# Enigmatisms/AdaPT

Hardware: AMD Instinct MI355X
Metric: Msamples/s (W*H*spp/s), unidirectional MIS path tracing (higher is better)
Workload: dtype f32

## Files before the change

adapt_amd/_lib.py:

```python
from __future__ import annotations

import ctypes as C
import os

_HERE = os.path.dirname(os.path.abspath(__file__))
LIB_PATHS = {"fast": os.environ.get("ADAPT_MI_LIB") or os.path.join(_HERE, "libadapt_mi.so"),
             "exact": os.environ.get("ADAPT_MI_LIB_EXACT") or os.path.join(_HERE, "libadapt_mi_exact.so")}
_variant = "exact" if os.environ.get("APT_EXACT", "0") not in ("", "0") else "fast"
LIB_PATH = LIB_PATHS[_variant]

f32p = C.POINTER(C.c_float)
i32p = C.POINTER(C.c_int32)
u32p = C.POINTER(C.c_uint32)
u8p = C.POINTER(C.c_uint8)
f64p = C.POINTER(C.c_double)
APT_N_KERNELS = 5
KERNEL_NAMES = ("generate", "extend", "shade", "shadow", "finalize")


class AptError(RuntimeError):
    pass


class SceneDesc(C.Structure):
# ... 85 lines not shown
    "apt_stream": (C.c_int, [C.c_void_p, C.POINTER(C.c_void_p)]),
    "apt_intersect": (C.c_int, [C.c_void_p, C.c_int32, f32p, f32p, i32p, f32p, f32p]),
    "apt_occluded": (C.c_int, [C.c_void_p, C.c_int32, f32p, f32p, f32p, i32p]),
    "apt_rng_stream": (C.c_int, [C.c_int32, C.c_uint32, C.c_uint32, C.c_uint32, C.c_int32, u32p]),
    "apt_bxdf_probe": (C.c_int, [C.c_int32, C.c_int32, i32p, f32p, f32p, C.c_float, C.c_int32, C.c_uint32, f32p]),
    "apt_medium_probe": (C.c_int, [C.c_int32, C.c_int32, i32p, f32p, C.c_int32, f32p, C.c_uint32, f32p]),
    "apt_volume_probe": (C.c_int, [C.c_int32, C.c_int32, i32p, f32p, f32p, C.c_int32, f32p, C.c_uint32, f32p]),
    "apt_emitter_probe": (C.c_int, [C.c_void_p, C.c_int32, f32p, C.c_uint32, f32p]),
    "apt_texture_probe": (C.c_int, [C.c_void_p, C.c_int32, i32p, f32p, f32p]),
    "apt_surface_maps_probe": (C.c_int, [C.c_void_p, C.c_int32, i32p, f32p, f32p]),
    "apt_transient_bin_probe": (C.c_int, [C.c_int32, C.c_int32, f32p, C.c_float, C.c_float, C.c_int32, i32p]),
    "apt_renderer_info": (C.c_int, [C.c_void_p, i32p, i32p, C.POINTER(C.c_int64), i32p, C.POINTER(C.c_char_p), i32p]),
    "apt_renderer_camera_fused": (C.c_int, [C.c_void_p, i32p]),
    "apt_renderer_light_strips": (C.c_int, [C.c_void_p, i32p]),
    "apt_renderer_record_staged": (C.c_int, [C.c_void_p, i32p]),
    "apt_measure_sclk_mhz": (C.c_int, [C.c_int32, f32p]),
    "apt_last_error": (C.c_char_p, []),
    "apt_version": (C.c_char_p, []),
}

_libs = {}


def use(variant: str) -> str:
    global _variant, LIB_PATH
    if variant not in LIB_PATHS:
        raise ValueError(f"unknown build variant {variant!r}")
    prev, _variant = _variant, variant
    LIB_PATH = LIB_PATHS[variant]
    return prev
# ... 36 lines not shown
```

adapt_amd/csrc/api.hip:

```cpp
#include <hip/hip_runtime.h>
#include <chrono>

#include <algorithm>
#include <cmath>
#include <cstdio>
#include <cstdlib>
#include <cstring>
#include <limits>
#include <memory>
#include <string>
#include <vector>

#include "../../include/adapt_mi.h"
#include "bvh_build.hpp"
#include "shade_stage.hpp"
#include "unit_kernels.hpp"
#include "aov.hpp"
#include "volumetric.hpp"

#define APT_EXPORT extern "C" __attribute__((visibility("default")))

static thread_local std::string g_err;
static int fail(int code, const std::string& msg) { g_err = msg; return code; }
#define HIP_TRY(expr)                                                                              \
    do {                                                                                           \
        hipError_t e_ = (expr);                                                                    \
        if (e_ != hipSuccess)                                                                      \
            return fail(APT_E_HIP, std::string(#expr) + ": " + hipGetErrorString(e_));             \
    } while (0)

typedef void (*shade_fn)(DevScene, Params, Queues, Counters*, ShadeIn, int, int);
typedef void (*shade_traced_fn)(DevScene, Params, Queues, Counters*, int, int);
typedef void (*shade_cam_fn)(DevScene, Params, Queues, Counters*, const unsigned long long*);
typedef void (*shade_tr_fn)(DevScene, Params, Queues, Counters*, ShadeIn, int, int, TransQ);
struct ShadeVariant { int bm, sm; const char* name; shade_fn fn; shade_tr_fn transient; shade_traced_fn traced; shade_cam_fn traced_cam; shade_traced_fn traced_staged; };
#if APT_FAST
#define APT_FLAT_FN(...) __VA_ARGS__
#else
#define APT_FLAT_FN(...) nullptr
#endif
#define APT_TRACED_PAIR(STEM, ...) APT_FLAT_FN(STEM<__VA_ARGS__>), APT_FLAT_FN(STEM##_cam<__VA_ARGS__>)
#define APT_TRACED_PLAIN(BM, SM, TEX) APT_TRACED_PAIR(k_shade_traced, BM, SM, TEX), nullptr
#define APT_TRACED_LEAN(BM, SM, TEX) APT_TRACED_PAIR(k_shade_traced_lean, BM, SM), APT_FLAT_FN(k_shade_traced_lean_staged<BM, SM>)
#define APT_SHADE_VARIANT(BM, SM, TEX, NAME, TRACED) {BM, SM, NAME, k_shade<BM, SM, TEX>, k_shade_tr<BM, SM, TEX>, APT_TRACED_##TRACED(BM, SM, TEX)}
static const ShadeVariant kShadeVariants[] = {
    APT_SHADE_VARIANT(APT_BX_LAMBERTIAN, APT_SRC_POINT, 0, "lambertian/point", LEAN),
    APT_SHADE_VARIANT(APT_BX_BLINN_PHONG | APT_BX_LAMBERTIAN, APT_SRC_POINT_AREA, 0, "phong+lambertian/point+area", PLAIN),
    APT_SHADE_VARIANT(APT_BX_BLINN_PHONG | APT_BX_LAMBERTIAN | APT_BX_MIRROR | APT_BX_GLASS, APT_SRC_POINT_AREA, 0, "phong+lambertian+mirror+glass/point+area", PLAIN),
    APT_SHADE_VARIANT(APT_BX_ALL, APT_SRC_ALL, 0, "all models", PLAIN),
};
static const ShadeVariant kTexturedShade = APT_SHADE_VARIANT(APT_BX_ALL, APT_SRC_ALL, 1, "all models + image textures", PLAIN);
struct ClassDef { int mask; const char* name; int group, slot, vgroup, vslot; };
constexpr int APT_N_GROUPS = 2, APT_N_VGROUPS = 3, APT_VGROUP_SLOTS = 4;
static constexpr ClassDef kClass[] = {
    {APT_BX_LAMBERTIAN, "lambertian", 0, 0, 0, 0},
    {APT_BX_BLINN_PHONG, "blinn-phong", 1, 0, 2, 0},
    {APT_BX_OREN_NAYAR, "oren-nayar", 1, 1, 0, 1},
    {APT_BX_MIRROR | APT_BX_GLASS | APT_BX_NULL, "delta", 0, 1, 0, 2},
// ... 134 lines not shown
enum Pipeline { PIPE_STAGED, PIPE_SORTED, PIPE_TRACED, PIPE_VOLUMETRIC };

struct apt_renderer {
    const apt_scene* scene = nullptr;
    apt_render_cfg cfg{};
    Params par{};
    int n_cols = 0, npix = 0, spp_batch = 1;
    int cnt = 0;
    std::vector<Lane> lanes;
    int n_lanes = 1;
    hipStream_t stream() const { return lanes[0].stream; }
    DevBuf accum, scratch, pix_key;
    DevBuf cam_strips;
    int record_stage = 0;
    shade_traced_fn traced_fn = nullptr;
    int camera_fuse = 0;
    int light_strips = 0;
    Counters host_counters{};
    int grid_small = 0, grid_trace = 0, nq = APT_MAX_NQ;
    const ShadeVariant* shade = nullptr;
    int trace_mode = TRACE_BVH;
    int trace_nt = BLOCK;
    int trace_items = BLOCK;
    Pipeline pipeline = PIPE_STAGED;
    int dyn_fetch = 0;
    bool tile_ok = false;
    extend_fn extend = nullptr, fix = nullptr;
    int ovf_levels = 0;
    int n_cq = 0;
    int vev_single = 0;
// ... 526 lines not shown
    if (textured) r->shade = &kTexturedShade;
    const char* env_sorted = getenv("APT_SORTED");
    const bool fits = sc->n_classes <= APT_MAX_CLASSES;
    const bool sorted = !textured && fits && (env_sorted ? (atoi(env_sorted) != 0 && sc->n_classes >= 1) : sc->n_classes >= 2);
    bool want_traced = true;
    if (const char* f = getenv("APT_FUSED")) {
        const int want = atoi(f);
        if (want == 1) fprintf(stderr, "adapt_mi: APT_FUSED=1 (light samples only traced in place) was retired in round 5; running the staged pipeline (APT_FUSED=0). Use 2 for rays traced in place.\n");
        want_traced = want >= 2;
    }
    const bool can_trace = r->trace_mode == TRACE_FLAT && S == 1 && !r->split() && r->shade->traced != nullptr;
    r->pipeline = c.volumetric ? PIPE_VOLUMETRIC : (sorted ? PIPE_SORTED : ((can_trace && want_traced) ? PIPE_TRACED : PIPE_STAGED));
    p.traced = (r->pipeline == PIPE_TRACED) ? 1 : 0;
    const bool want_stage = !(getenv("APT_RECORD_STAGE") && atoi(getenv("APT_RECORD_STAGE")) == 0);
    r->record_stage = (p.traced && want_stage && r->shade->traced_staged != nullptr) ? 1 : 0;
    r->traced_fn = r->record_stage ? r->shade->traced_staged : r->shade->traced;
    p.nee_vm = (!c.volumetric && !r->split() && r->trace_mode == TRACE_FLAT && S > 1) ? 1 : 0;
    p.l_planes = (!p.nee_vm && S >= 2 && S <= 4) ? S : 1;
    if (r->pipeline == PIPE_VOLUMETRIC) {
        if (c.max_bounce > 255) { return fail(APT_E_INVALID, "apt_renderer_create: the volumetric tracer keeps the bounce count in 8 bits (max_bounce <= 255)"); }
        if (!sc->has_aabb) { return fail(APT_E_INVALID, "apt_renderer_create: the volumetric tracer needs the object boxes (world bound)"); }
        r->vev_single = (textured || sc->n_classes + 1 > APT_MAX_CLASSES) ? 1 : 0;
        const int n_surf = r->vev_single ? 1 : sc->n_classes;
        r->n_cq = n_surf + 1;
        const int smi = vgroup_emitter_set(sc->src_mask), vi = sc->has_volume ? 1 : 0;
        r->vev_all = kVEventAll[smi][vi];
        for (size_t o = 0; o < sc->obj_class.size(); o++)
            if (!sc->obj_null[o]) r->vev_live[r->vev_single ? 0 : sc->obj_class[o]] = true;
        r->vev_live[n_surf] = true;
        for (int g = 0; g < APT_N_VGROUPS; g++) { r->vgroup_fn[g] = kVGroup[smi][vi][g]; for (int k = 0; k < APT_VGROUP_SLOTS; k++) r->vgroup_cls[g][k] = -1; }
        if (!r->vev_single) for (int c = 0; c < n_surf; c++) if (r->vev_live[c]) r->vgroup_cls[kClass[sc->class_def[c]].vgroup][kClass[sc->class_def[c]].vslot] = c;
// ... 524 lines not shown
    const int batch_cap = lane_batch(r, n_spp);
    while (done < n_spp) {
        const int B = (n_spp - done < batch_cap) ? (n_spp - done) : batch_cap;
        Lane& ln = r->lanes[(size_t)(batch % r->n_lanes)];
        hipStream_t st = ln.stream;
        const Queues& q = ln.q;
        Counters* cnt = ln.cnt();
        Params p = r->par; p.cnt_base = r->cnt; p.spp_batch = B;
        const size_t total = (size_t)r->npix * (size_t)B;
        if (int rc = begin_batch(r, ln)) return rc;
#if APT_FAST
        if (r->pipeline == PIPE_TRACED) {
            const unsigned long long* strips = r->cam_strips.as<unsigned long long>();
            int cur = 0, b0 = 0;
            if (r->camera_fuse) {
                { LaunchTimer t(r, APT_K_SHADE, st); hipLaunchKernelGGL(r->shade->traced_cam, dim3(grid_for(total, r->grid_small, nq)), dim3(BLOCK), 0, st, sc, p, q, cnt, strips); }
                { LaunchTimer t(r, APT_K_SHADE, st); hipLaunchKernelGGL(r->traced_fn, dim3(r->grid_fix), dim3(BLOCK), 0, st, sc, p, q, cnt, 0, 0); }
                cur = 1; b0 = 1;
            } else {
                LaunchTimer t(r, APT_K_GENERATE, st);
                if (r->adaptive) hipLaunchKernelGGL(k_generate_trace_ad, dim3(grid_for(total, r->grid_small, 1)), dim3(BLOCK), 0, st, sc, p, q, cnt, (const uint8_t*)r->aq.active, strips);
                else hipLaunchKernelGGL(k_generate_trace, dim3(grid_for(total, r->grid_small, 1)), dim3(BLOCK), 0, st, sc, p, q, cnt, strips);
            }
            for (int b = b0; b < p.max_bounce; b++) {
                { LaunchTimer t(r, APT_K_SHADE, st); hipLaunchKernelGGL(r->traced_fn, dim3(grid_for(total, r->grid_small, nq)), dim3(BLOCK), 0, st, sc, p, q, cnt, cur, b); }
                cur ^= 1;
            }
            if (p.max_bounce > 0) { LaunchTimer t(r, APT_K_SHADOW, st, false); hipLaunchKernelGGL(r->fix, dim3(r->grid_fix), dim3(BLOCK), 0, st, sc, p, q, cnt, cur, (const uint32_t*)cnt->n_active[cur], ln.plan); }
        } else
#endif
        {
// ... 593 lines not shown
APT_EXPORT int apt_renderer_camera_fused(const apt_renderer* r, int32_t* out) {
    if (!r || !out) return fail(APT_E_INVALID, "apt_renderer_camera_fused: null argument");
    *out = r->camera_fuse;
    return APT_OK;
}
APT_EXPORT int apt_renderer_light_strips(const apt_renderer* r, int32_t* out) {
    if (!r || !out) return fail(APT_E_INVALID, "apt_renderer_light_strips: null argument");
    *out = r->light_strips;
    return APT_OK;
}
APT_EXPORT int apt_renderer_record_staged(const apt_renderer* r, int32_t* out) {
    if (!r || !out) return fail(APT_E_INVALID, "apt_renderer_record_staged: null argument");
    *out = r->record_stage;
    return APT_OK;
}
APT_EXPORT int apt_renderer_info(const apt_renderer* r, int32_t* spp_batch, int32_t* n_subqueues, int64_t* queue_bytes, int32_t* lds_bytes, const char** shade_variant, int32_t* trace_mode) {
    if (!r) return fail(APT_E_INVALID, "apt_renderer_info: null handle");
    if (spp_batch) *spp_batch = r->spp_batch;
    if (n_subqueues) *n_subqueues = r->nq;
    if (queue_bytes) *queue_bytes = (int64_t)r->lanes[0].pool.bytes * (int64_t)r->lanes.size();
    if (lds_bytes) *lds_bytes = (int32_t)r->lds_bytes;
    if (shade_variant) *shade_variant = r->shade_name.c_str();
    if (trace_mode) *trace_mode = r->trace_mode;
    return APT_OK;
}
```

adapt_amd/csrc/shade_stage.hpp:

```cpp
#pragma once
#include "stages.hpp"

APT_D float ti_fmod(float a, float b) { float q = floorf(a / b); return a - b * q; }
APT_D f3 mix3(f3 a, f3 b, float t) { return a * (1.0f - t) + b * t; }
APT_D f3 texture_query(const DevScene& sc, int map, int obj, float u, float v) {
    const int* ti_ = sc.tex_i + 15 * obj + 5 * map; const float* tf = sc.tex_f + 6 * obj + 2 * map;
    const float w = (float)ti_[3], h = (float)ti_[4];
    const float scaled_u = ti_fmod((u * tf[0]) * w, w - 1.f), scaled_v = ti_fmod((v * tf[1]) * h, h - 1.f);
    float floor_u = floorf(scaled_u), floor_v = floorf(scaled_v);
    const float ratio_u = fmaxf(scaled_u - floor_u, 0.f), ratio_v = fmaxf(scaled_v - floor_v, 0.f);
    floor_u = fminf(fmaxf(floor_u, 0.f), w - 1.f); floor_v = fminf(fmaxf(floor_v, 0.f), h - 1.f);
    const float ceil_u = fminf(floor_u + 1.f, w - 1.f), ceil_v = fminf(floor_v + 1.f, h - 1.f);
    const int fu = (int)(floor_u + (float)ti_[1]), fv = (int)(floor_v + (float)ti_[2]), cu = (int)(ceil_u + (float)ti_[1]), cv = (int)(ceil_v + (float)ti_[2]);
    const float* img = sc.atlas[map]; const int W = sc.atlas_w[map];
    const float* r0 = img + (size_t)fv * W * 3; const float* r1 = img + (size_t)cv * W * 3;
    const f3 q_ff = ld3(r0 + 3 * fu), q_cf = ld3(r0 + 3 * cu), q_fc = ld3(r1 + 3 * fu), q_cc = ld3(r1 + 3 * cu);
    return mix3(mix3(q_ff, q_cf, ratio_u), mix3(q_fc, q_cc, ratio_u), ratio_v);
}
APT_D bool get_uv_item(const DevScene& sc, int map, int obj, int prim, float bu, float bv, f3& out) {
    if (sc.atlas[map] == nullptr || !(sc.tex_i[15 * obj + 5 * map] > -255)) return false;
    const float* uv = sc.uvs + 6 * prim;
    const float w0 = 1.f - bu - bv;
    const float gu = (uv[2] * bu + uv[4] * bv) + uv[0] * w0, gv = (uv[3] * bu + uv[5] * bv) + uv[1] * w0;
    out = texture_query(sc, map, obj, gu, gv);
// ... 185 lines not shown
    ls.contrib = (c * (A_->p).inv_S) * vx.thr;
    ls.want = !(ls.contrib.x == 0.f && ls.contrib.y == 0.f && ls.contrib.z == 0.f);
    return ls;
}
template <int BM, int SM, typename R, typename Gather>
APT_D f3 emit_and_scatter(const ShadeArgs3* A_, Vertex& vx, R& rng, float& new_pdf, bool& is_spec, Gather&& gather) {
    if ((SM & APT_SRC_AREA) && vx.hit_light >= 0) {
        const f3 emit_int = emitter_eval_le((A_->sc).src[vx.hit_light], vx.hit_point - vx.o, vx.it.n_s);
        if (!(emit_int.x == 0.f && emit_int.y == 0.f && emit_int.z == 0.f)) gather((emit_int * vx.emission_weight) * vx.thr);
    }
    f3 spec;
    const f3 new_d = surface_sample<BM>(vx.bx, vx.it, vx.d, (A_->sc).world_ior, (A_->p).two_sides, rng, spec, new_pdf, is_spec);
    vx.thr = vx.thr * fdiv3(spec, new_pdf);
    return new_d;
}
APT_D void shadow_store(const Queues& q, uint32_t so, f3 o, f3 dir, float dist, f3 contrib) {
    st3q(q.sh_o, q.sh_cap, so, o); st3q(q.sh_d, q.sh_cap, so, dir); stq(q.sh_tmax, so, dist); st3q(q.sh_c, q.sh_cap, so, contrib);
}
struct ShadeTally { uint32_t shade, shadow, poison; };
APT_D void tally_flush(const ShadeTally& t, const uint32_t* s_draws, Counters* cnt, int sq) {
    flush_uniform(t.shade, &cnt->stats[sq][ST_SHADE]);
    flush_uniform(t.shadow, &cnt->stats[sq][ST_SHADOW]);
    if (lane_id() == 0 && s_draws[threadIdx.x >> 6]) atomicAdd(&cnt->stats[sq][ST_DRAWS], (unsigned long long)s_draws[threadIdx.x >> 6]);
    flush_uniform(t.poison, &cnt->stats[sq][ST_POISON]);
}
#if APT_FAST
template <int BM, int SM, int TEX, bool CAM = false, bool STAGE = false>
APT_D void shade_traced(args3_ptr A0, Counters* cnt, int cur_, int bounce_, const unsigned long long* strips = nullptr) {
    static_assert(!(CAM && STAGE), "a camera-fed row loads no record");
    const ShadeArgs3* A_ = args_fresh(A0);
    const int cur = CAM ? 0 : cur_, bounce = CAM ? 0 : bounce_;
    const int nxt = cur ^ 1;
    const SubLoop sl = sub_loop((A_->p).nq);
    const uint32_t qbase = (uint32_t)sl.q * (A_->p).subcap, sh_qbase = (uint32_t)sl.q * (A_->q).sh_subcap;
    uint32_t* next_counter = &cnt->n_tr[(bounce + 1) % 3][0][sl.q * CNT_PAD];
    if (sl.first == 0 && threadIdx.x == 0) {
        cnt->n_tr[(bounce + 2) % 3][0][sl.q * CNT_PAD] = 0;
        cnt->n_tr[(bounce + 2) % 3][(A_->q).tr_ncls][sl.q * CNT_PAD] = 0;
    }
    const EmitterGeom geom = {(A_->sc).precom, (A_->sc).normals, (A_->sc).obj_info};
    __shared__ uint32_t s_draws[BLOCK / 64];
    if (lane_id() == 0) s_draws[threadIdx.x >> 6] = 0;
    ShadeTally tl = {0u, 0u, 0u};
    uint32_t t_traced = 0, t_lit = 0, t_extend = 0, t_samples = 0;
// ... 48 lines not shown
#ifdef APT_ROWTOP_STATS
    t_loop0 = __builtin_amdgcn_s_memtime();
#endif
    for (uint32_t base = sl.first; base < n; base += sl.stride) {
        APT_ARGS_PHASE();
        const uint32_t pos = base + threadIdx.x, idx = qbase + pos;
        bool alive = pos < n;
        const uint32_t cu_pm = pf_pm;
        float4 cu_ra = make_float4(0.f, 0.f, 0.f, 0.f), cu_rb = cu_ra;
        if (PFP) { const int rp = max(tr_prim(cu_pm), 0); cu_ra = (A_->sc).prim_shade[2 * rp]; cu_rb = (A_->sc).prim_shade[2 * rp + 1]; prefetch_prim(base + sl.stride); }
        Vertex vx; vertex_reset(vx);
        Rng rng; rng_init(rng, 0u, 0u, 0u, 0u);
        f3 Lc = splat3(0.f);
        bool entry = alive;
        float ray_pdf = 1.f;
        if constexpr (CAM) {
            const uint32_t w = (uint32_t)__builtin_amdgcn_readfirstlane((int)(pos >> 6)) * (uint32_t)(A_->p).nq + (uint32_t)sl.q;
            const uint32_t id_ = w * 64u + lane_id();
            const bool valid = alive && id_ < cam_total;
            f3 dir = mk3(0.f, 0.f, 1.f);
            uint32_t draws = 0;
            uint32_t jitter_tail[2] = {0u, 0u};
            if (valid) {
                const uint32_t lp = id_ % (uint32_t)(A_->p).npix, s = id_ / (uint32_t)(A_->p).npix;
                int i, j; local_to_global((A_->p), lp, i, j);
                for (int pl = 0; pl < (A_->p).l_planes; pl++) stL((A_->q).L, (A_->p).cap, (id_ << 2) | (uint32_t)pl, splat3(0.f));
                dir = camera_ray_dir((A_->p), i, j, s, draws, WINDOW ? jitter_tail : nullptr);
                vx.id = (s << (A_->p).pix_bits) | lp;
            }
            if (draws) atomicAdd(&s_draws[threadIdx.x >> 6], draws);
            const f3 cam_o = mk3((A_->p).cam_t[0], (A_->p).cam_t[1], (A_->p).cam_t[2]);
// ... 19 lines not shown
                }
            }
            entry = valid && !c_defer;
            alive = entry && hr.prim >= 0;
            if (alive) {
                vx.o = cam_o; vx.d = dir; vx.thr = splat3(1.f);
                f3 rec_kd; float2 uv; uv.x = hr.u; uv.y = hr.v;
                build_hit((A_->sc), hr.prim, hr.t, uv.x, uv.y, vx.o, vx.d, vx.it, vx.hit_light, rec_kd);
                alive = open_vertex<BM, SM, TEX>(A_, vx, rng, hr.prim, rec_kd, tr_meta(tr_pack(hr.prim, draws, false), 0u), ray_pdf, uv, 0, WINDOW ? jitter_tail : nullptr);
            }
        }
        rec4 sa = {0.f, 0.f, 0.f, 0.f}, sb = sa, sc_ = sa, sd = sa;
        if constexpr (STAGE) {
            staged_read(s_rec + lane_id(), sa, sb, sc_, sd);
            { const int rp = max(tr_prim(__float_as_uint(sb.w)), 0); rec4 pa, pb; staged_read2(s_prim + 2 * rp, pa, pb); cu_ra = make_float4(pa.x, pa.y, pa.z, pa.w); cu_rb = make_float4(pb.x, pb.y, pb.z, pb.w); }
            if (alive && bounce > 0) { Lc = mk3(sd.x, sd.y, sd.z); if (SM & APT_SRC_AREA) ray_pdf = sd.w; }
        }
        if (!CAM && !STAGE && alive && bounce > 0) { const float4 dd = ldq(trD, idx << 4); Lc = mk3(dd.x, dd.y, dd.z); if (SM & APT_SRC_AREA) ray_pdf = dd.w; }
        if (!CAM && alive) {
            float4 a, b_, c;
            if constexpr (STAGE) { a = make_float4(sa.x, sa.y, sa.z, sa.w); b_ = make_float4(sb.x, sb.y, sb.z, sb.w); c = make_float4(sc_.x, sc_.y, sc_.z, sc_.w); }
            else { a = ldq(trA, idx << 4); b_ = ldq(trB, idx << 4); c = ldq(trC, idx << 4); }
#ifdef APT_ROWTOP_STATS
            if constexpr (!STAGE) { const unsigned long long t0_ = __builtin_amdgcn_s_memtime(); staged_wait(); t_rowtop += __builtin_amdgcn_s_memtime() - t0_; t_rows++; }
#endif
            vx.o = mk3(a.x, a.y, a.z); vx.d = mk3(b_.x, b_.y, b_.z); vx.thr = mk3(c.x, c.y, c.z); vx.id = __float_as_uint(c.w);
            const uint32_t pm = PFP ? cu_pm : __float_as_uint(b_.w);
            const int prim = tr_prim(pm);
            if (prim < 0) alive = false;
            else {
                f3 rec_kd; float2 uv; uv.x = uv.y = 0.f;
                if ((A_->sc).has_vn || (TEX && (A_->sc).tex_i != nullptr)) uv = ldq((A_->q).tr_uv[cur], idx << 3);
                if (PFP || STAGE) build_hit_rec((A_->sc), cu_ra, cu_rb, prim, a.w, uv.x, uv.y, vx.o, vx.d, vx.it, vx.hit_light, rec_kd);
                else build_hit((A_->sc), prim, a.w, uv.x, uv.y, vx.o, vx.d, vx.it, vx.hit_light, rec_kd);
                alive = open_vertex<BM, SM, TEX>(A_, vx, rng, prim, rec_kd, tr_meta(pm, (uint32_t)bounce), ray_pdf, uv, bounce);
            }
        }
        tl.shade += wave_count(alive);
#ifdef APT_NEAR_STATS
        t_near += wave_count(alive && bounce > 0 && vx.it.min_depth < 2e-3f);
#endif
        if (alive) vx.hit_point = vx.d * vx.it.min_depth + vx.o;

        APT_ARGS_PHASE();
        bool break_flag = false;
        DevSrc src_only;
        if ((A_->sc).n_sources == 1) src_only = ld_src_uniform((A_->sc).src);
        const LightSample f = sample_light<BM, SM, false>(A_, vx, rng, geom, src_only, alive, break_flag);
        if (f.poisoned) Lc = splat3(f.mis_w);
        tl.shadow += wave_count(f.sampled); tl.poison += wave_count(f.poisoned);
        int occ_e = 0;
        if ((A_->sc).n_sources != 1) {
            const unsigned long long wm = __ballot(f.want);
            occ_e = -1;
            if (wm != 0ull) {
                const int e0 = __builtin_amdgcn_readlane(f.src, __ffsll((long long)wm) - 1);
                if (!__any(f.want && f.src != e0)) occ_e = e0;
            }
        }
        if constexpr (STAGE) if (base + sl.stride < n) stage_row(base + sl.stride);
        APT_ARGS_PHASE();
        bool cont = false, is_spec = false;
        f3 new_d = mk3(0.f, 1.f, 0.f);
        float new_pdf = 1.f;
        if (alive) {
            new_d = emit_and_scatter<BM, SM>(A_, vx, rng, new_pdf, is_spec, [&](f3 add) { Lc = Lc + add; });
            cont = (bounce + 1) < (A_->p).max_bounce;
        }
        if (rng.draw != vx.draw0) {
            if constexpr (STAGE) lds_add_unordered(&s_draws[threadIdx.x >> 6], rng.draw - vx.draw0);
            else atomicAdd(&s_draws[threadIdx.x >> 6], rng.draw - vx.draw0);
        }
        APT_ARGS_PHASE();
        float tr_t = 0.f; int tr_hit = -1; float tr_u = 0.f, tr_v = 0.f; int tr_q = -1;
        TrAppend tr_app; tr_app.raw = 0u; tr_app.rank = 0u;
        {
            int tr_idx = -1, tr_run = -1, hit_cls = 0;
            if (__any(cont)) tr_idx = flat_closest1((A_->sc).flat, vx.hit_point, new_d, 1e7f, tr_t, tr_run);
            const bool tr_defer = cont && (tr_run >= 0 || flat_needs_cull((A_->sc).flat, new_d));
            t_extend += wave_count(cont);
            cont = cont && (tr_idx >= 0 || tr_defer);
            if (cont && !tr_defer) { HitRec hr; flat_resolve((A_->sc).flat, tr_idx, tr_t, vx.hit_point, new_d, hr, hit_cls); tr_hit = hr.prim; tr_u = hr.u; tr_v = hr.v; }
            tr_q = !cont ? -1 : (tr_defer ? 1 : 0);
            { const Append a_ = append_issue(tr_q == 0, next_counter); tr_app.raw = a_.raw; tr_app.rank = rank_in(a_.m); }
// ... 192 lines not shown
template <int BM, int SM, int TEX = 0>
__global__ void __launch_bounds__(BLOCK) k_shade_traced(DevScene sc, Params p, Queues q, Counters* cnt, int cur, int bounce) {
    shade_traced<BM, SM, TEX>(kernel_args3(), cnt, cur, bounce);
}
#ifndef APT_TRACED_WAVES
#define APT_TRACED_WAVES 7
#endif
template <int BM, int SM>
__global__ void __launch_bounds__(BLOCK) __attribute__((amdgpu_waves_per_eu(APT_TRACED_WAVES, APT_TRACED_WAVES))) k_shade_traced_lean(DevScene sc, Params p, Queues q, Counters* cnt, int cur, int bounce) {
    shade_traced<BM, SM, 0>(kernel_args3(), cnt, cur, bounce);
}
template <int BM, int SM>
__global__ void __launch_bounds__(BLOCK) __attribute__((amdgpu_waves_per_eu(APT_TRACED_WAVES, APT_TRACED_WAVES))) k_shade_traced_lean_staged(DevScene sc, Params p, Queues q, Counters* cnt, int cur, int bounce) {
    shade_traced<BM, SM, 0, false, true>(kernel_args3(), cnt, cur, bounce);
}
template <int BM, int SM, int TEX = 0>
__global__ void __launch_bounds__(BLOCK) k_shade_traced_cam(DevScene sc, Params p, Queues q, Counters* cnt, const unsigned long long* strips) {
    shade_traced<BM, SM, TEX, true>(kernel_args3(), cnt, 0, 0, strips);
}
#ifndef APT_TRACED_CAM_WAVES
#define APT_TRACED_CAM_WAVES 7
#endif
template <int BM, int SM>
__global__ void __launch_bounds__(BLOCK) __attribute__((amdgpu_waves_per_eu(APT_TRACED_CAM_WAVES, APT_TRACED_CAM_WAVES))) k_shade_traced_lean_cam(DevScene sc, Params p, Queues q, Counters* cnt, const unsigned long long* strips) {
    shade_traced<BM, SM, 0, true>(kernel_args3(), cnt, 0, 0, strips);
}
#endif

#define APT_GROUP_SLOTS 6
struct GroupIn { const uint32_t* counts[APT_GROUP_SLOTS]; int cls[APT_GROUP_SLOTS]; };
template <int SM, int WAVES, int B0, int B1, int B2, int B3, int B4 = 0, int B5 = 0>
__global__ void __launch_bounds__(BLOCK, WAVES) k_shade_group(DevScene sc, Params p, Queues q, Counters* cnt, GroupIn g, int cur, int bounce) {
    ShadeIn in = {nullptr, nullptr, nullptr, nullptr, nullptr, nullptr, nullptr, nullptr, nullptr, nullptr, nullptr, 0};
    if constexpr (B0 != 0) if (g.cls[0] >= 0) { in.counts = g.counts[0]; in.cls = g.cls[0]; shade_staged<B0, SM, 0, true>(kernel_args3(), cnt, in, cur, bounce); }
    if constexpr (B1 != 0) if (g.cls[1] >= 0) { in.counts = g.counts[1]; in.cls = g.cls[1]; shade_staged<B1, SM, 0, true>(kernel_args3(), cnt, in, cur, bounce); }
    if constexpr (B2 != 0) if (g.cls[2] >= 0) { in.counts = g.counts[2]; in.cls = g.cls[2]; shade_staged<B2, SM, 0, true>(kernel_args3(), cnt, in, cur, bounce); }
    if constexpr (B4 != 0) if (g.cls[4] >= 0) { in.counts = g.counts[4]; in.cls = g.cls[4]; shade_staged<B4, SM, 0, true>(kernel_args3(), cnt, in, cur, bounce); }
    if constexpr (B5 != 0) if (g.cls[5] >= 0) { in.counts = g.counts[5]; in.cls = g.cls[5]; shade_staged<B5, SM, 0, true>(kernel_args3(), cnt, in, cur, bounce); }
    if constexpr (B3 != 0) if (g.cls[3] >= 0) { in.counts = g.counts[3]; in.cls = g.cls[3]; shade_staged<B3, SM, 0, true>(kernel_args3(), cnt, in, cur, bounce); }
}
// ... 11 lines not shown
```

adapt_amd/renderer.py:

```python
from __future__ import annotations

import ctypes as C
import time
from typing import List, Optional

import numpy as np

from . import _lib
from .scene_pack import FlatScene, RenderConfig, make_config, pack_scene
from .tiles import TilePlan

__all__ = ["Renderer", "VolumeRenderer", "DeviceScene", "bxdf_probe", "medium_probe", "volume_probe", "rng_stream", "adaptive_config", "adaptive_segments", "relative_error", "DENOISE_DEFAULTS"]

ADAPTIVE_DEFAULTS = {"min_spp": 64, "step": 32}
DENOISE_DEFAULTS = {"firefly_threshold": 0.0, "iterations": 3, "sigma_n": 128.0, "sigma_z": 0.1, "sigma_a": 0.1, "sigma_c": 1.0, "demodulate": True}
TRAVERSAL_NAMES = dict(enumerate(("bvh", "sweep", "tile", "flat")))
BVH_BUILDER_NAMES = dict(enumerate(("sah", "lbvh", "ploc")))


def adaptive_config(adaptive) -> Optional[dict]:
    if adaptive is None or adaptive is False:
        return None
    if not isinstance(adaptive, dict):
        raise TypeError("adaptive must be None or a dict {'threshold': t, 'min_spp': 64, 'step': 32}")
# ... 499 lines not shown
    def camera_fused(self) -> bool:
        f = C.c_int32(0)
        _lib.check(self.lib.apt_renderer_camera_fused(self.handle, C.byref(f)), "apt_renderer_camera_fused", self.lib)
        return bool(f.value)

    def light_strips(self) -> bool:
        f = C.c_int32(0)
        _lib.check(self.lib.apt_renderer_light_strips(self.handle, C.byref(f)), "apt_renderer_light_strips", self.lib)
        return bool(f.value)

    def record_staged(self) -> bool:
        f = C.c_int32(0)
        _lib.check(self.lib.apt_renderer_record_staged(self.handle, C.byref(f)), "apt_renderer_record_staged", self.lib)
        return bool(f.value)

    def get_check_point(self) -> dict:
        return {"w": self.w, "h": self.h, "crop_x": self.crop_x, "crop_y": self.crop_y, "crop_rx": self.crop_rx,
                "crop_ry": self.crop_ry, "focal": self.focal, "num_objects": self.num_objects, "num_prims": self.num_prims,
                "cam_orient": np.array(self.cam_orient), "src_num": self.src_num, "cam_t": np.array(self.cam_t),
                "accumulation": self.color.to_numpy(), "counter": self._cnt,
                **({"transient_bins": self.tile_transient()} if self.n_bins else {}),
                **({"path_length_planes": self.tile_path_lengths()} if self.n_lengths else {}),
                **({"aov_sums": self.tile_aov(), "aov_samples": self._aov_n} if self._aov_n else {}),
                **(self._adaptive_check_point() if self.adaptive else {})}

    _ADAPTIVE_KEYS = ("adaptive", "sample_counts", "moments", "active")

    def _adaptive_check_point(self) -> dict:
        n, act = self.tile_sample_counts(with_mask=True)
        return {"adaptive": dict(self.adaptive), "sample_counts": n, "moments": self.tile_moments(), "active": act}
# ... 57 lines not shown
```

include/adapt_mi.h:

```cpp
#ifndef ADAPT_MI_H
#define ADAPT_MI_H

#include <stdint.h>

#ifdef __cplusplus
extern "C" {
#endif

#define APT_OK            0
#define APT_E_INVALID    -1
#define APT_E_NO_DEVICE  -2
#define APT_E_HIP        -3
#define APT_E_NOMEM      -4
#define APT_E_STATE      -5

typedef struct apt_bvh apt_bvh;
typedef struct apt_scene apt_scene;
typedef struct apt_renderer apt_renderer;

typedef struct apt_scene_desc {
    int32_t n_prims, n_objects, n_sources, has_vertex_normal;
    const float*   prims;
    const float*   normals;
    const float*   v_normals;
// ... 133 lines not shown
int apt_bxdf_probe(int32_t device, int32_t n, const int32_t* bxdf_i, const float* bxdf_f, const float* dirs12,
                   float world_ior, int32_t do_sample, uint32_t seed, float* out);
int apt_texture_probe(const apt_scene*, int32_t n, const int32_t* map_obj, const float* uv, float* out3);
int apt_surface_maps_probe(const apt_scene*, int32_t n, const int32_t* prim_first, const float* bary, float* out7);
int apt_medium_probe(int32_t device, int32_t n, const int32_t* med_i, const float* med_f, int32_t mode, const float* in7,
                     uint32_t seed, float* out8);
int apt_volume_probe(int32_t device, int32_t n, const int32_t* vol_i, const float* vol_f, const float* vol_grid, int32_t mode,
                     const float* in10, uint32_t seed, float* out8);
int apt_emitter_probe(const apt_scene*, int32_t n, const float* in11, uint32_t seed, float* out12);
int apt_transient_bin_probe(int32_t device, int32_t n, const float* t, float min_time, float interval, int32_t n_bins, int32_t* out);
int apt_renderer_info(const apt_renderer*, int32_t* spp_batch, int32_t* n_subqueues, int64_t* queue_bytes,
                      int32_t* lds_bytes, const char** shade_variant, int32_t* trace_mode);
int apt_renderer_camera_fused(const apt_renderer*, int32_t* fused);
int apt_renderer_light_strips(const apt_renderer*, int32_t* in_use);
int apt_renderer_record_staged(const apt_renderer*, int32_t* staged);

int apt_measure_sclk_mhz(int32_t device, float* mhz);

const char* apt_last_error(void);
const char* apt_version(void);

#ifdef __cplusplus
}
#endif
#endif
```

Before: 6298.

## Add live-row variants of lean traced shade kernels with wave-uniform RNG windows

Adds staged and camera-fed 'live' variants of the lean Lambertian/point traced shade kernel. They open each vertex through a draw window that is only evaluated when any lane in the wave is still alive. They also run light sampling and scatter on every lane unconditionally rather than behind per-lane alive branches, and update draw counts once per path. The aim is to cut divergence and per-lane branching in the shading rows. The cost is extra code paths and redundant arithmetic on dead lanes. The variants are selected by default when the renderer uses the traced pipeline, with an environment variable to turn them off.

```diff
diff --git a/adapt_amd/_lib.py b/adapt_amd/_lib.py
--- a/adapt_amd/_lib.py
+++ b/adapt_amd/_lib.py
@@ -123,6 +123,7 @@
     "apt_renderer_camera_fused": (C.c_int, [C.c_void_p, i32p]),
     "apt_renderer_light_strips": (C.c_int, [C.c_void_p, i32p]),
     "apt_renderer_record_staged": (C.c_int, [C.c_void_p, i32p]),
+    "apt_renderer_live_rows": (C.c_int, [C.c_void_p, i32p]),
     "apt_measure_sclk_mhz": (C.c_int, [C.c_int32, f32p]),
     "apt_last_error": (C.c_char_p, []),
     "apt_version": (C.c_char_p, []),
diff --git a/adapt_amd/csrc/api.hip b/adapt_amd/csrc/api.hip
--- a/adapt_amd/csrc/api.hip
+++ b/adapt_amd/csrc/api.hip
@@ -33,15 +33,15 @@
 typedef void (*shade_traced_fn)(DevScene, Params, Queues, Counters*, int, int);
 typedef void (*shade_cam_fn)(DevScene, Params, Queues, Counters*, const unsigned long long*);
 typedef void (*shade_tr_fn)(DevScene, Params, Queues, Counters*, ShadeIn, int, int, TransQ);
-struct ShadeVariant { int bm, sm; const char* name; shade_fn fn; shade_tr_fn transient; shade_traced_fn traced; shade_cam_fn traced_cam; shade_traced_fn traced_staged; };
+struct ShadeVariant { int bm, sm; const char* name; shade_fn fn; shade_tr_fn transient; shade_traced_fn traced; shade_cam_fn traced_cam; shade_traced_fn traced_staged, traced_staged_live; shade_cam_fn traced_cam_live; };
 #if APT_FAST
 #define APT_FLAT_FN(...) __VA_ARGS__
 #else
 #define APT_FLAT_FN(...) nullptr
 #endif
 #define APT_TRACED_PAIR(STEM, ...) APT_FLAT_FN(STEM<__VA_ARGS__>), APT_FLAT_FN(STEM##_cam<__VA_ARGS__>)
-#define APT_TRACED_PLAIN(BM, SM, TEX) APT_TRACED_PAIR(k_shade_traced, BM, SM, TEX), nullptr
-#define APT_TRACED_LEAN(BM, SM, TEX) APT_TRACED_PAIR(k_shade_traced_lean, BM, SM), APT_FLAT_FN(k_shade_traced_lean_staged<BM, SM>)
+#define APT_TRACED_PLAIN(BM, SM, TEX) APT_TRACED_PAIR(k_shade_traced, BM, SM, TEX), nullptr, nullptr, nullptr
+#define APT_TRACED_LEAN(BM, SM, TEX) APT_TRACED_PAIR(k_shade_traced_lean, BM, SM), APT_FLAT_FN(k_shade_traced_lean_staged<BM, SM>), APT_FLAT_FN(k_shade_traced_lean_staged_live<BM, SM>), APT_FLAT_FN(k_shade_traced_lean_cam_live<BM, SM>)
 #define APT_SHADE_VARIANT(BM, SM, TEX, NAME, TRACED) {BM, SM, NAME, k_shade<BM, SM, TEX>, k_shade_tr<BM, SM, TEX>, APT_TRACED_##TRACED(BM, SM, TEX)}
 static const ShadeVariant kShadeVariants[] = {
     APT_SHADE_VARIANT(APT_BX_LAMBERTIAN, APT_SRC_POINT, 0, "lambertian/point", LEAN),
@@ -206,6 +206,8 @@
     DevBuf cam_strips;
     int record_stage = 0;
     shade_traced_fn traced_fn = nullptr;
+    int live_rows = 0;
+    shade_cam_fn traced_cam_fn = nullptr;
     int camera_fuse = 0;
     int light_strips = 0;
     Counters host_counters{};
@@ -762,7 +764,10 @@
     p.traced = (r->pipeline == PIPE_TRACED) ? 1 : 0;
     const bool want_stage = !(getenv("APT_RECORD_STAGE") && atoi(getenv("APT_RECORD_STAGE")) == 0);
     r->record_stage = (p.traced && want_stage && r->shade->traced_staged != nullptr) ? 1 : 0;
-    r->traced_fn = r->record_stage ? r->shade->traced_staged : r->shade->traced;
+    const bool want_live = !(getenv("APT_LIVE_ROWS") && atoi(getenv("APT_LIVE_ROWS")) == 0);
+    r->live_rows = (p.traced && want_live && r->shade->traced_staged_live != nullptr && r->shade->traced_cam_live != nullptr) ? 1 : 0;
+    r->traced_fn = r->record_stage ? (r->live_rows ? r->shade->traced_staged_live : r->shade->traced_staged) : r->shade->traced;
+    r->traced_cam_fn = r->live_rows ? r->shade->traced_cam_live : r->shade->traced_cam;
     p.nee_vm = (!c.volumetric && !r->split() && r->trace_mode == TRACE_FLAT && S > 1) ? 1 : 0;
     p.l_planes = (!p.nee_vm && S >= 2 && S <= 4) ? S : 1;
     if (r->pipeline == PIPE_VOLUMETRIC) {
@@ -1317,7 +1322,7 @@
             const unsigned long long* strips = r->cam_strips.as<unsigned long long>();
             int cur = 0, b0 = 0;
             if (r->camera_fuse) {
-                { LaunchTimer t(r, APT_K_SHADE, st); hipLaunchKernelGGL(r->shade->traced_cam, dim3(grid_for(total, r->grid_small, nq)), dim3(BLOCK), 0, st, sc, p, q, cnt, strips); }
+                { LaunchTimer t(r, APT_K_SHADE, st); hipLaunchKernelGGL(r->traced_cam_fn, dim3(grid_for(total, r->grid_small, nq)), dim3(BLOCK), 0, st, sc, p, q, cnt, strips); }
                 { LaunchTimer t(r, APT_K_SHADE, st); hipLaunchKernelGGL(r->traced_fn, dim3(r->grid_fix), dim3(BLOCK), 0, st, sc, p, q, cnt, 0, 0); }
                 cur = 1; b0 = 1;
             } else {
@@ -1941,6 +1946,11 @@
     *out = r->record_stage;
     return APT_OK;
 }
+APT_EXPORT int apt_renderer_live_rows(const apt_renderer* r, int32_t* out) {
+    if (!r || !out) return fail(APT_E_INVALID, "apt_renderer_live_rows: null argument");
+    *out = r->live_rows;
+    return APT_OK;
+}
 APT_EXPORT int apt_renderer_info(const apt_renderer* r, int32_t* spp_batch, int32_t* n_subqueues, int64_t* queue_bytes, int32_t* lds_bytes, const char** shade_variant, int32_t* trace_mode) {
     if (!r) return fail(APT_E_INVALID, "apt_renderer_info: null handle");
     if (spp_batch) *spp_batch = r->spp_batch;
diff --git a/adapt_amd/csrc/shade_stage.hpp b/adapt_amd/csrc/shade_stage.hpp
--- a/adapt_amd/csrc/shade_stage.hpp
+++ b/adapt_amd/csrc/shade_stage.hpp
@@ -223,6 +223,56 @@
     vx.thr = vx.thr * fdiv3(spec, new_pdf);
     return new_d;
 }
+template <int BM, int SM>
+APT_D bool open_vertex_live(const ShadeArgs3* A_, Vertex& vx, DrawWindow& rng, f3 rec_kd, uint32_t pm, int bounce, bool alive, const uint32_t* jitter_tail = nullptr) {
+    static_assert(BM == APT_BX_LAMBERTIAN && !(SM & APT_SRC_AREA), "a draw window serves [roulette] index [index] u1 u2: Lambertian surfaces, emitters that draw nothing");
+    vx.bx.k_d = rec_kd;
+    const uint32_t lp = vx.id & ((1u << (A_->p).pix_bits) - 1u), s = vx.id >> (A_->p).pix_bits;
+    vx.l_off = (s * (uint32_t)(A_->p).npix + lp) << 2;
+    vx.draw0 = (pm >> 8) & 0xffffu;
+    const uint32_t key0 = ((A_->p).world == 1) ? lp : ldq((A_->p).pix_key, lp << 2), ctr0 = (uint32_t)((A_->p).cnt_base + (int)s + 1);
+    bool roulette = false; float mx = 0.f;
+    if ((A_->p).use_rr) { mx = max3(vx.thr); roulette = mx < (A_->p).rr_threshold && bounce >= (A_->p).rr_bounce_th; }
+    else alive = alive && !(max3(vx.thr) < 1e-4f);
+    const bool relight = vx.hit_light >= 0 && (A_->sc).n_sources > 1;
+    const bool have_first = jitter_tail != nullptr && (A_->p).anti_alias != 0;
+    uint32_t c[4] = {0u, 0u, have_first ? jitter_tail[0] : 0u, have_first ? jitter_tail[1] : 0u};
+    const bool live = window_open(rng, key0, (A_->p).seed, ctr0, vx.draw0, roulette, mx, relight, c, have_first, [alive](bool v) { return __any(v && alive) != 0; });
+    if (roulette) vx.thr = vx.thr * srcp(mx + 1e-7f);
+    return alive && live;
+}
+template <int BM, int SM, typename R>
+APT_D LightSample sample_light_live(const ShadeArgs3* A_, Vertex& vx, R& rng, const EmitterGeom& geom, const DevSrc src_only, bool active) {
+    LightSample ls;
+    const int ns = (A_->sc).n_sources;
+    int sidx = rng_int(rng);
+    sidx = (ns == 1) ? 0 : pymod(sidx, ns);
+    float emitter_pdf = (A_->p).inv_ns;
+    if (ns <= 1) active = active && vx.hit_light < 0;
+    else if (vx.hit_light >= 0) {
+        sidx = rng_int(rng);
+        sidx = (ns == 2) ? 0 : pymod(sidx, ns - 1);
+        if (sidx >= vx.hit_light) sidx += 1;
+        emitter_pdf = (A_->p).inv_ns1;
+    }
+    DevSrc src = src_only;
+    if (ns != 1) src = (A_->sc).src[sidx];
+    ls.src = sidx;
+    f3 shadow_int; float direct_pdf;
+    const f3 to_emitter = emitter_sample_hit<SM>(src, geom, vx.hit_point, rng, shadow_int, direct_pdf) - vx.hit_point;
+    ls.dist = fnorm(to_emitter);
+    ls.dir = fdiv3(to_emitter, ls.dist);
+    ls.sampled = active;
+    const f3 direct_spec = surface_eval<BM>(vx.bx, vx.it, vx.d, ls.dir, (A_->sc).world_ior, (A_->p).two_sides);
+    ls.mis_w = 1.0f;
+    if ((A_->p).use_mis && !(src.bool_bits & 0x01)) ls.mis_w = balance(emitter_pdf * direct_pdf, surface_pdf<BM>(vx.bx, vx.it, ls.dir, vx.d, (A_->sc).world_ior, (A_->p).two_sides));
+    ls.poisoned = active && isnan(ls.mis_w);
+    f3 c = (direct_spec * shadow_int) * ls.mis_w;
+    if (ns != 1) c = fdiv3(c, emitter_pdf);
+    ls.contrib = (c * (A_->p).inv_S) * vx.thr;
+    ls.want = active && !ls.poisoned && !(ls.contrib.x == 0.f && ls.contrib.y == 0.f && ls.contrib.z == 0.f);
+    return ls;
+}
 APT_D void shadow_store(const Queues& q, uint32_t so, f3 o, f3 dir, float dist, f3 contrib) {
     st3q(q.sh_o, q.sh_cap, so, o); st3q(q.sh_d, q.sh_cap, so, dir); stq(q.sh_tmax, so, dist); st3q(q.sh_c, q.sh_cap, so, contrib);
 }
@@ -234,9 +284,11 @@
     flush_uniform(t.poison, &cnt->stats[sq][ST_POISON]);
 }
 #if APT_FAST
-template <int BM, int SM, int TEX, bool CAM = false, bool STAGE = false>
+template <int BM, int SM, int TEX, bool CAM = false, bool STAGE = false, bool LIVE_ = false>
 APT_D void shade_traced(args3_ptr A0, Counters* cnt, int cur_, int bounce_, const unsigned long long* strips = nullptr) {
     static_assert(!(CAM && STAGE), "a camera-fed row loads no record");
+    static_assert(!LIVE_ || ((CAM || STAGE) && TEX == 0), "live rows: the staged and the camera-fed form of the lean kernels");
+    constexpr bool LIVE = LIVE_ && APT_DRAW_WINDOW != 0;
     const ShadeArgs3* A_ = args_fresh(A0);
     const int cur = CAM ? 0 : cur_, bounce = CAM ? 0 : bounce_;
     const int nxt = cur ^ 1;
@@ -315,7 +367,49 @@
         f3 Lc = splat3(0.f);
         bool entry = alive;
         float ray_pdf = 1.f;
-        if constexpr (CAM) {
+        if constexpr (CAM && LIVE) {
+            const uint32_t w = (uint32_t)__builtin_amdgcn_readfirstlane((int)(pos >> 6)) * (uint32_t)(A_->p).nq + (uint32_t)sl.q;
+            const uint32_t id_ = w * 64u + lane_id();
+            const bool valid = alive && id_ < cam_total;
+            uint32_t draws = 0;
+            uint32_t jitter_tail[2] = {0u, 0u};
+            const uint32_t lp = id_ % (uint32_t)(A_->p).npix, s = id_ / (uint32_t)(A_->p).npix;
+            int i, j; local_to_global((A_->p), lp, i, j);
+            if (valid) for (int pl = 0; pl < (A_->p).l_planes; pl++) stL((A_->q).L, (A_->p).cap, (id_ << 2) | (uint32_t)pl, splat3(0.f));
+            const f3 dir = camera_ray_dir((A_->p), i, j, s, draws, WINDOW ? jitter_tail : nullptr);
+            vx.id = (s << (A_->p).pix_bits) | lp;
+            if (valid && draws) atomicAdd(&s_draws[threadIdx.x >> 6], draws);
+            const f3 cam_o = mk3((A_->p).cam_t[0], (A_->p).cam_t[1], (A_->p).cam_t[2]);
+            float c_t = 0.f; int c_run = -1, c_idx = -1;
+            if (__any(valid)) c_idx = flat_closest1<true>((A_->sc).flat, cam_o, dir, 1e7f, c_t, c_run, camera_strip_mask((A_->p), strips, w));
+            const bool c_defer = valid && (c_run >= 0 || flat_needs_cull((A_->sc).flat, dir));
+            HitRec hr; int hit_cls = 0;
+            flat_resolve((A_->sc).flat, max(c_idx, 0), c_t, cam_o, dir, hr, hit_cls);
+            { const uint32_t nv = wave_count(valid); t_samples += nv; t_extend += nv; }
+            if (__any(c_defer)) {
+                const int ncls = (A_->q).tr_ncls;
+                const uint32_t dpos = wave_append(c_defer, &cnt->n_tr[0][ncls][sl.q * CNT_PAD]);
+                if (c_defer) {
+                    const uint32_t slot = (A_->q).tr_stage_top ? qbase + (A_->p).subcap - 1u - dpos : (uint32_t)ncls * (A_->p).cap + qbase + dpos, so = slot << 4;
+                    float one = 1.f, far_ = 1e7f, zero = 0.f;
+                    asm volatile("" : "+v"(one), "+v"(far_), "+v"(zero));
+                    stq((A_->q).tr[0][0], so, make_float4(cam_o.x, cam_o.y, cam_o.z, far_));
+                    stq((A_->q).tr[0][1], so, make_float4(dir.x, dir.y, dir.z, __uint_as_float(tr_pack(-1, draws, false))));
+                    stq((A_->q).tr[0][2], so, make_float4(one, one, one, __uint_as_float(vx.id)));
+                    stq((A_->q).tr[0][3], so, make_float4(zero, zero, zero, one));
+                    if ((A_->sc).has_vn || (A_->sc).tex_i != nullptr) { float2 uv_; uv_.x = zero; uv_.y = zero; stq((A_->q).tr_uv[0], slot << 3, uv_); }
+                }
+            }
+            entry = valid && !c_defer;
+            alive = entry && c_idx >= 0 && hr.prim >= 0;
+            vx.o = cam_o; vx.d = dir; vx.thr = splat3(1.f);
+            f3 rec_kd;
+            build_hit((A_->sc), max(hr.prim, 0), hr.t, hr.u, hr.v, vx.o, vx.d, vx.it, vx.hit_light, rec_kd);
+            const bool opened = alive;
+            alive = open_vertex_live<BM, SM>(A_, vx, rng, rec_kd, tr_pack(hr.prim, draws, false), 0, alive, WINDOW ? jitter_tail : nullptr);
+            if (opened && !alive && rng.draw != vx.draw0) atomicAdd(&s_draws[threadIdx.x >> 6], rng.draw - vx.draw0);
+        }
+        if constexpr (CAM && !LIVE) {
             const uint32_t w = (uint32_t)__builtin_amdgcn_readfirstlane((int)(pos >> 6)) * (uint32_t)(A_->p).nq + (uint32_t)sl.q;
             const uint32_t id_ = w * 64u + lane_id();
             const bool valid = alive && id_ < cam_total;
@@ -365,10 +459,23 @@
         if constexpr (STAGE) {
             staged_read(s_rec + lane_id(), sa, sb, sc_, sd);
             { const int rp = max(tr_prim(__float_as_uint(sb.w)), 0); rec4 pa, pb; staged_read2(s_prim + 2 * rp, pa, pb); cu_ra = make_float4(pa.x, pa.y, pa.z, pa.w); cu_rb = make_float4(pb.x, pb.y, pb.z, pb.w); }
-            if (alive && bounce > 0) { Lc = mk3(sd.x, sd.y, sd.z); if (SM & APT_SRC_AREA) ray_pdf = sd.w; }
+            if constexpr (!LIVE) if (alive && bounce > 0) { Lc = mk3(sd.x, sd.y, sd.z); if (SM & APT_SRC_AREA) ray_pdf = sd.w; }
+        }
+        if constexpr (LIVE && STAGE) {
+            if (bounce > 0) Lc = mk3(sd.x, sd.y, sd.z);
+            vx.o = mk3(sa.x, sa.y, sa.z); vx.d = mk3(sb.x, sb.y, sb.z); vx.thr = mk3(sc_.x, sc_.y, sc_.z); vx.id = __float_as_uint(sc_.w);
+            const uint32_t pm = __float_as_uint(sb.w);
+            const int prim = tr_prim(pm);
+            alive = alive && prim >= 0;
+            f3 rec_kd; float2 uv; uv.x = uv.y = 0.f;
+            if ((A_->sc).has_vn) { if (alive) uv = ldq((A_->q).tr_uv[cur], idx << 3); }
+            build_hit_rec((A_->sc), cu_ra, cu_rb, max(prim, 0), sa.w, uv.x, uv.y, vx.o, vx.d, vx.it, vx.hit_light, rec_kd);
+            const bool opened = alive;
+            alive = open_vertex_live<BM, SM>(A_, vx, rng, rec_kd, pm, bounce, alive);
+            if (opened && !alive && rng.draw != vx.draw0) lds_add_unordered(&s_draws[threadIdx.x >> 6], rng.draw - vx.draw0);
         }
         if (!CAM && !STAGE && alive && bounce > 0) { const float4 dd = ldq(trD, idx << 4); Lc = mk3(dd.x, dd.y, dd.z); if (SM & APT_SRC_AREA) ray_pdf = dd.w; }
-        if (!CAM && alive) {
+        if (!CAM && !LIVE && alive) {
             float4 a, b_, c;
             if constexpr (STAGE) { a = make_float4(sa.x, sa.y, sa.z, sa.w); b_ = make_float4(sb.x, sb.y, sb.z, sb.w); c = make_float4(sc_.x, sc_.y, sc_.z, sc_.w); }
             else { a = ldq(trA, idx << 4); b_ = ldq(trB, idx << 4); c = ldq(trC, idx << 4); }
@@ -391,13 +498,15 @@
 #ifdef APT_NEAR_STATS
         t_near += wave_count(alive && bounce > 0 && vx.it.min_depth < 2e-3f);
 #endif
-        if (alive) vx.hit_point = vx.d * vx.it.min_depth + vx.o;
+        if (LIVE || alive) vx.hit_point = vx.d * vx.it.min_depth + vx.o;
 
         APT_ARGS_PHASE();
         bool break_flag = false;
         DevSrc src_only;
         if ((A_->sc).n_sources == 1) src_only = ld_src_uniform((A_->sc).src);
-        const LightSample f = sample_light<BM, SM, false>(A_, vx, rng, geom, src_only, alive, break_flag);
+        LightSample f;
+        if constexpr (LIVE) f = sample_light_live<BM, SM>(A_, vx, rng, geom, src_only, alive);
+        else f = sample_light<BM, SM, false>(A_, vx, rng, geom, src_only, alive, break_flag);
         if (f.poisoned) Lc = splat3(f.mis_w);
         tl.shadow += wave_count(f.sampled); tl.poison += wave_count(f.poisoned);
         int occ_e = 0;
@@ -414,11 +523,18 @@
         bool cont = false, is_spec = false;
         f3 new_d = mk3(0.f, 1.f, 0.f);
         float new_pdf = 1.f;
-        if (alive) {
+        if constexpr (LIVE) {
+            if ((bounce + 1) < (A_->p).max_bounce) { new_d = emit_and_scatter<BM, SM>(A_, vx, rng, new_pdf, is_spec, [&](f3 add) { Lc = Lc + add; }); cont = alive; }
+            else rng.draw += 2u;
+            if (alive) {
+                if constexpr (STAGE) lds_add_unordered(&s_draws[threadIdx.x >> 6], rng.draw - vx.draw0);
+                else atomicAdd(&s_draws[threadIdx.x >> 6], rng.draw - vx.draw0);
+            }
+        } else if (alive) {
             new_d = emit_and_scatter<BM, SM>(A_, vx, rng, new_pdf, is_spec, [&](f3 add) { Lc = Lc + add; });
             cont = (bounce + 1) < (A_->p).max_bounce;
         }
-        if (rng.draw != vx.draw0) {
+        if (!LIVE && rng.draw != vx.draw0) {
             if constexpr (STAGE) lds_add_unordered(&s_draws[threadIdx.x >> 6], rng.draw - vx.draw0);
             else atomicAdd(&s_draws[threadIdx.x >> 6], rng.draw - vx.draw0);
         }
@@ -641,6 +757,10 @@
 __global__ void __launch_bounds__(BLOCK) __attribute__((amdgpu_waves_per_eu(APT_TRACED_WAVES, APT_TRACED_WAVES))) k_shade_traced_lean_staged(DevScene sc, Params p, Queues q, Counters* cnt, int cur, int bounce) {
     shade_traced<BM, SM, 0, false, true>(kernel_args3(), cnt, cur, bounce);
 }
+template <int BM, int SM>
+__global__ void __launch_bounds__(BLOCK) __attribute__((amdgpu_waves_per_eu(APT_TRACED_WAVES, APT_TRACED_WAVES))) k_shade_traced_lean_staged_live(DevScene sc, Params p, Queues q, Counters* cnt, int cur, int bounce) {
+    shade_traced<BM, SM, 0, false, true, true>(kernel_args3(), cnt, cur, bounce);
+}
 template <int BM, int SM, int TEX = 0>
 __global__ void __launch_bounds__(BLOCK) k_shade_traced_cam(DevScene sc, Params p, Queues q, Counters* cnt, const unsigned long long* strips) {
     shade_traced<BM, SM, TEX, true>(kernel_args3(), cnt, 0, 0, strips);
@@ -651,6 +771,10 @@
 template <int BM, int SM>
 __global__ void __launch_bounds__(BLOCK) __attribute__((amdgpu_waves_per_eu(APT_TRACED_CAM_WAVES, APT_TRACED_CAM_WAVES))) k_shade_traced_lean_cam(DevScene sc, Params p, Queues q, Counters* cnt, const unsigned long long* strips) {
     shade_traced<BM, SM, 0, true>(kernel_args3(), cnt, 0, 0, strips);
+}
+template <int BM, int SM>
+__global__ void __launch_bounds__(BLOCK) __attribute__((amdgpu_waves_per_eu(APT_TRACED_CAM_WAVES, APT_TRACED_CAM_WAVES))) k_shade_traced_lean_cam_live(DevScene sc, Params p, Queues q, Counters* cnt, const unsigned long long* strips) {
+    shade_traced<BM, SM, 0, true, false, true>(kernel_args3(), cnt, 0, 0, strips);
 }
 #endif
 
diff --git a/adapt_amd/renderer.py b/adapt_amd/renderer.py
--- a/adapt_amd/renderer.py
+++ b/adapt_amd/renderer.py
@@ -537,6 +537,11 @@
         _lib.check(self.lib.apt_renderer_record_staged(self.handle, C.byref(f)), "apt_renderer_record_staged", self.lib)
         return bool(f.value)
 
+    def live_rows(self) -> bool:
+        f = C.c_int32(0)
+        _lib.check(self.lib.apt_renderer_live_rows(self.handle, C.byref(f)), "apt_renderer_live_rows", self.lib)
+        return bool(f.value)
+
     def get_check_point(self) -> dict:
         return {"w": self.w, "h": self.h, "crop_x": self.crop_x, "crop_y": self.crop_y, "crop_rx": self.crop_rx,
                 "crop_ry": self.crop_ry, "focal": self.focal, "num_objects": self.num_objects, "num_prims": self.num_prims,
diff --git a/include/adapt_mi.h b/include/adapt_mi.h
--- a/include/adapt_mi.h
+++ b/include/adapt_mi.h
@@ -171,6 +171,7 @@
 int apt_renderer_camera_fused(const apt_renderer*, int32_t* fused);
 int apt_renderer_light_strips(const apt_renderer*, int32_t* in_use);
 int apt_renderer_record_staged(const apt_renderer*, int32_t* staged);
+int apt_renderer_live_rows(const apt_renderer*, int32_t* live);
 
 int apt_measure_sclk_mhz(int32_t device, float* mhz);
 
```

After: 6430, median of 6. +2.1%, better.
